# pjmikkol/bwtc

Hardware: NVIDIA B200
Metric: forward BWT MB/s (SA+BWT, 32 MiB blocks) (higher is better)
Workload: dtype u8 text / u32 ranks / u64 sort keys (integer)

## Files before the change

bwtc_b200/csrc/bwt_engine.cu:

```cuda
#include "../../include/bwtc_cuda.h"
#include "bwt_kernels.cuh"
#include "ibwt_kernels.cuh"

#include <algorithm>
#include <atomic>
#include <chrono>
#include <cmath>
#include <condition_variable>
#include <cstdarg>
#include <cstdio>
#include <cstdlib>
#include <cstring>
#include <deque>
#include <memory>
#include <mutex>
#include <thread>
#include <unordered_map>
#include <vector>

using namespace bwtc_b200;

namespace {

constexpr int RS_BLOCK = BWTC_RS_BLOCK;
// ... 46 lines not shown
  bool ring_busy[RING_SLOTS] = {false, false, false, false};
  int poll_spin_us = 150, poll_sleep_us = 40;
  int wait_mode = 0;
  uint32_t cap = 0;
  size_t max_rs_tiles = 0, max_aux_tiles = 0;
  uint8_t* d_in = nullptr;
  uint8_t* d_text = nullptr;
  uint8_t* d_out = nullptr;
  uint32_t* d_rank = nullptr;
  void* d_keys[2] = {nullptr, nullptr};
  uint32_t* d_idx[2] = {nullptr, nullptr};
  uint8_t* d_aux[2] = {nullptr, nullptr};
  uint32_t* d_scat = nullptr;
  uint32_t* d_zero = nullptr;
  uint32_t* d_status = nullptr;
  uint32_t* d_tilecnt = nullptr;
  uint32_t* d_LF = nullptr;
  uint32_t* d_livebits = nullptr;
  uint32_t* d_ktab = nullptr;
  LookupParams* d_lookup = nullptr;
  LookupParams* h_lookup = nullptr;
  LadderState* d_state = nullptr;
  LadderState* h_state = nullptr;
  unsigned long long* d_wtab = nullptr;
  uint32_t* d_bhist = nullptr;
  const uint8_t** d_bptr = nullptr;
  int32_t* d_sa = nullptr;
  uint32_t* h_small = nullptr;
  uint8_t* h_batch = nullptr;
  cudaEvent_t ev_begin = nullptr, ev_end = nullptr;
  std::vector<cudaEvent_t> ev_pool;
  int timing_detail = 0;
  int static_tiles = 1;
  int lb_watchdog = 0;
  int debug_fake_watchdog = 0;
  int debug_reverse_tiles = 0;
  int verify = 0;
  int debug_corrupt_out = 0;
  uint32_t debug_corrupt_lf = 0;
  int64_t debug_corrupt_sa = -1;
  int d2h_kernel = 0;
  int d2h_ctas = 16;
  int debug_skip_copies = 0;
  int ladder_first = 2, ladder_more = 4;
  int use_radix9 = 0;
  uint32_t status_row_words = 256;
  int use_partial = 1;
  int use_gram = 1;
  int twopass = 0;
  int hybrid2 = 0;
  uint32_t rerank_pf_tiles = 0;
  int use_lazy = 1;
  uint32_t lazy_min_suffixes = 4u << 20;
  double lazy_max_live = 0.065;
  int use_seg = 1;
  int use_batch = 1;
  int use_pack_pred = 1;
  uint32_t aux_min_suffixes = 96u << 20;
  int bucket_min_windows = 3;
  uint64_t rerank_window_bytes = 72ull << 20;
  uint32_t force_chars = 0, force_keybytes = 0;
  uint32_t debug_max_rounds = 0;
  int last_cur = 0;
  RerankParams rr0;
  bwtc_cuda_stats stats;
  char err[512];
  uint32_t* d_ctrl() const { return d_zero; }
  uint32_t* d_hist() const { return d_zero + CTR_WORDS; }
  unsigned long long* d_tstate() const { return reinterpret_cast<unsigned long long*>(d_zero + CTR_WORDS + HIST_WORDS); }
  uint32_t* h_ctrl() const { return h_small; }
  uint32_t* h_hist() const { return h_small + CTR_WORDS; }
  uint32_t* h_LF() const { return h_small + CTR_WORDS + HIST_WORDS; }
};

#define CK(ctx, call)                                                                              \
  do {                                                                                             \
    cudaError_t e_ = (call);                                                                       \
    if (e_ != cudaSuccess) {                                                                       \
      set_err((ctx)->err, "CUDA error %s at %s:%d: %s", cudaGetErrorName(e_), __FILE__, __LINE__,  \
              cudaGetErrorString(e_));                                                             \
      return BWTC_CUDA_ECUDA;                                                                      \
    }                                                                                              \
  } while (0)

namespace {

template <typename KeyT, int IPT, bool IOTA, bool AUX, int RB = 8>
int set_pass_attr(bwtc_cuda_ctx* ctx) {
  CK(ctx, cudaFuncSetAttribute(k_radix_pass<KeyT, RS_BLOCK, IPT, IOTA, AUX, RB>, cudaFuncAttributeMaxDynamicSharedMemorySize,
                               (int)RadixPassSmem<KeyT, RS_BLOCK, IPT, AUX, RB>::bytes));
  return 0;
}

void ctx_free(bwtc_cuda_ctx* c) {
  if (!c) return;
  cudaSetDevice(c->device);
  if (c->stream) cudaStreamSynchronize(c->stream);
  cudaFree(c->d_in); cudaFree(c->d_text); cudaFree(c->d_out); cudaFree(c->d_rank);
  cudaFree(c->d_keys[0]); cudaFree(c->d_keys[1]); cudaFree(c->d_idx[0]); cudaFree(c->d_idx[1]);
  cudaFree(c->d_zero); cudaFree(c->d_status); cudaFree(c->d_LF); cudaFree(c->d_wtab); cudaFree(c->d_tilecnt); cudaFree(c->d_scat);
  cudaFree(c->d_bhist); cudaFree(c->d_bptr); cudaFree(c->d_aux[0]); cudaFree(c->d_aux[1]);
  cudaFree(c->d_state); cudaFree(c->d_livebits); cudaFree(c->d_ktab); cudaFree(c->d_lookup); cudaFree(c->d_sa);
  if (c->h_lookup) cudaFreeHost(c->h_lookup);
  if (c->h_batch) cudaFreeHost(c->h_batch);
  if (c->h_small) cudaFreeHost(c->h_small);
  if (c->h_state) cudaFreeHost(c->h_state);
  if (c->h_ring) cudaFreeHost(c->h_ring);
  if (c->ev_begin) cudaEventDestroy(c->ev_begin);
  if (c->ev_end) cudaEventDestroy(c->ev_end);
  if (c->ev_sync) cudaEventDestroy(c->ev_sync);
  if (c->ev_in) cudaEventDestroy(c->ev_in);
  if (c->ev_comp) cudaEventDestroy(c->ev_comp);
  for (cudaEvent_t e : c->ev_ring) if (e) cudaEventDestroy(e);
  for (cudaEvent_t e : c->ev_pool) cudaEventDestroy(e);
  if (c->s_in) cudaStreamDestroy(c->s_in);
  if (c->s_out) cudaStreamDestroy(c->s_out);
  if (c->stream) cudaStreamDestroy(c->stream);
  delete c;
}

struct Round0Plan {
  uint32_t sigma, bits, chars, keybytes, npass;
  uint32_t rb;
  uint32_t rbits;
  PackParams pp;
  bool has_memory;
  double live_pred;
};

void plan_round0(const bwtc_cuda_ctx* ctx, const uint64_t* count, const bool* present, uint32_t N,
                 const double* pair_stats, Round0Plan* pl, uint32_t blk_bits = 0) {
  uint32_t sigma = blk_bits ? 1u : 0u;
  double total = 0, H0 = 0;
  for (int c = 0; c < 256; ++c) {
    pl->pp.lut[c] = 0;
    if (present[c]) { pl->pp.lut[c] = (uint8_t)sigma; ++sigma; total += (double)count[c]; }
  }
  if (sigma > 256) sigma = 256;
  for (int c = 0; c < 256; ++c)
    if (present[c] && count[c]) { double p = (double)count[c] / total; H0 -= p * std::log2(p); }
  const uint32_t b = sigma <= 2 ? 1 : ceil_log2_u64(sigma);
  const uint32_t cmax64 = (64 - blk_bits) / b, cmax32 = blk_bits >= 32 - b ? 0u : (32 - blk_bits) / b;
  uint32_t chars, keybytes;
  if (ctx->force_chars || ctx->force_keybytes) {
    keybytes = (ctx->force_keybytes == 4 && cmax32 >= 1) ? 4 : 8;
    const uint32_t cmax = keybytes == 4 ? cmax32 : cmax64;
    chars = ctx->force_chars ? ctx->force_chars : cmax;
    if (chars > cmax) chars = cmax;
    if (chars < 1) chars = 1;
  } else {
    double q2 = 0.0;
    for (int c = 0; c < 256; ++c)
      if (present[c] && count[c]) { const double q = (double)count[c] / total; q2 += q * q; }
    const double samples = pair_stats[1];
    const double all_pairs = samples * (samples - 1.0) * 0.5;
    const double expected = all_pairs * std::pow(q2, 8.0);
    const bool has_memory = (H0 < 1e-3) || samples < 64.0 || (pair_stats[0] > 8.0 * expected + 16.0);
    if (has_memory) {
      keybytes = 8;
      chars = cmax64;
    } else {
      const double npd = std::ceil((2.0 * std::log2((double)N + 2.0)) / 8.0);
      double best = 1e300;
      chars = cmax64;
      for (uint32_t c = 1; c <= cmax64; ++c) {
        const double p0 = std::ceil(((double)c * b + blk_bits) / 8.0) * ((uint64_t)c * b + blk_bits > 32 ? 1.1 : 1.0);
        const double L = 1.0 - std::exp(-(double)N * std::exp2(-H0 * (double)c));
        const double cost = p0 + L * (npd + 2.0);
        if (cost < best - 1e-9) { best = cost; chars = c; }
      }
      const uint32_t np = div_up((uint64_t)chars * b + blk_bits, 8);
      const uint32_t cfull = (8 * np - blk_bits) / b;
      const uint32_t cap = ((uint64_t)chars * b + blk_bits <= 32) ? cmax32 : cmax64;
      chars = cfull < cap ? cfull : cap;
      keybytes = ((uint64_t)chars * b + blk_bits <= 32) ? 4 : 8;
    }
  }
  pl->has_memory = true;
  pl->live_pred = 1.0;
  if (!(ctx->force_chars || ctx->force_keybytes)) {
    double q2 = 0.0;
    for (int c = 0; c < 256; ++c)
      if (present[c] && count[c]) { const double q = (double)count[c] / total; q2 += q * q; }
    const double samples = pair_stats[1];
    const double expected = samples * (samples - 1.0) * 0.5 * std::pow(q2, 8.0);
    pl->has_memory = (H0 < 1e-3) || samples < 64.0 || (pair_stats[0] > 8.0 * expected + 16.0);
    if (!pl->has_memory) pl->live_pred = 1.0 - std::exp(-(double)N * std::exp2(-H0 * (double)chars));
  }
  pl->sigma = sigma;
  pl->bits = b;
  pl->chars = chars;
  pl->keybytes = keybytes;
  pl->npass = div_up((uint64_t)chars * b + blk_bits, 8);
  pl->rb = 8;
  if (ctx->use_radix9 && keybytes == 8 && div_up((uint64_t)chars * b + blk_bits, 9) < pl->npass) {
    pl->rb = 9;
    pl->npass = div_up((uint64_t)chars * b + blk_bits, 9);
  }
  {
    const uint32_t covered = std::min<uint32_t>(pl->rb * pl->npass, keybytes * 8u);
    const uint32_t used = chars * b + blk_bits;
    uint32_t r = (ctx->use_partial && blk_bits == 0 && covered > used) ? covered - used : 0u;
    if (r >= b) r = b - 1u;
    if (chars >= 64u) r = 0;
    pl->rbits = r;
  }
  pl->pp.rbits = pl->rbits;
  pl->pp.bits = b;
  pl->pp.chars = chars;
  pl->pp.nblocks = 1;
  pl->pp.stride = 0;
}

uint32_t rerank_windows(const bwtc_cuda_ctx* ctx, uint32_t N, uint32_t m) {
  if ((uint64_t)m * 4 < (uint64_t)N) return 1;
  uint64_t w = ((uint64_t)N * 4 + ctx->rerank_window_bytes - 1) / ctx->rerank_window_bytes;
  if (w < 1) w = 1;
  if (!ctx->bucket_min_windows && w > 8) w = 8;
  if (w > MAX_RERANK_WINDOWS) w = MAX_RERANK_WINDOWS;
  return (uint32_t)w;
}

uint32_t rerank_launches(const bwtc_cuda_ctx* ctx, uint32_t N, uint32_t m) {
  const uint32_t w = rerank_windows(ctx, N, m);
  return (ctx->bucket_min_windows && w >= (uint32_t)ctx->bucket_min_windows) ? 1u : w;
}

inline bool dbg_any(const bwtc_cuda_ctx* ctx) { return ctx->debug_max_rounds != 0; }

inline uint32_t tile_slot(const bwtc_cuda_ctx* ctx, uint32_t ticket_word) {
  if (!ctx->static_tiles) return ticket_word;
  return ctx->debug_reverse_tiles ? CTR_STATIC_REV : CTR_STATIC;
}

inline uint32_t* status_rows(const bwtc_cuda_ctx* ctx, int p) {
  return ctx->d_status + ((size_t)p * (ctx->max_rs_tiles + LB_PAD_ROWS) + LB_PAD_ROWS) * ctx->status_row_words;
}

struct PassTimer {
  bwtc_cuda_ctx* ctx;
// ... 517 lines not shown
        }
        if (sft >= 32u) use_gram = false;
        gp.u[p] = (uint8_t)u;
        gp.s[p] = (uint8_t)sft;
      }
      gp.npass = pl.npass;
    }
    uint32_t* gram = use_gram ? ctx->d_hist() + GRAM_OFF : nullptr;
    if (use_gram) { hist_mask = 0; dp.count = 0; }
    if (pl.keybytes == 4) {
      k_pack_round0<uint32_t><<<grid, 256, 0, st>>>(d_text, N, static_cast<uint32_t*>(ctx->d_keys[0]), pl.pp,
                                                     ctx->d_hist(), hist_mask, ptiles, pl.rb, gram);
      if (dp.count) k_hist_derive<uint32_t><<<dp.count, 256, 0, st>>>(d_text, N, pl.pp, dp, ctx->d_hist(), pl.rb);
      if (use_gram) k_hist_from_gram<uint32_t><<<gp.npass, 256, 0, st>>>(d_text, N, pl.pp, gp, gram, ctx->d_hist(), pl.rb);
    } else {
      k_pack_round0<unsigned long long><<<grid, 256, 0, st>>>(d_text, N, static_cast<unsigned long long*>(ctx->d_keys[0]),
                                                               pl.pp, ctx->d_hist(), hist_mask, ptiles, pl.rb, gram);
      if (dp.count) k_hist_derive<unsigned long long><<<dp.count, 256, 0, st>>>(d_text, N, pl.pp, dp, ctx->d_hist(), pl.rb);
      if (use_gram)
        k_hist_from_gram<unsigned long long><<<gp.npass, 256, 0, st>>>(d_text, N, pl.pp, gp, gram, ctx->d_hist(), pl.rb);
    }
    if (dp.count || use_gram) S.kernel_launches++;
    CK(ctx, cudaGetLastError());
    S.kernel_launches++;
    S.algorithmic_bytes += (uint64_t)N + (uint64_t)N * pl.keybytes;
  }
  const uint32_t mask0 = all0;
  int cur = 0;
  uint32_t pdone = 0;
  int rc;
  uint32_t id_bits = (uint32_t)ceil_log2_u64((uint64_t)N);
  if (id_bits < 1) id_bits = 1;
  const bool pack_pred = ctx->use_pack_pred && (id_bits + pl.bits <= 32) && (mask0 & 1u);
  const uint32_t topshift = (pl.chars - 1) * pl.bits + pl.rbits;
  const uint32_t pred_mask = (1u << pl.bits) - 1u;
  const bool aux_pred = !pack_pred && ctx->aux_min_suffixes && N >= ctx->aux_min_suffixes && (mask0 & 1u) && !bs;
  if (pl.keybytes == 4)
    rc = run_sort<uint32_t, RS_IPT32>(ctx, N, mask0, true, N - 1, &cur, &pt, &pdone, pack_pred ? id_bits : 0u, topshift,
                                      pred_mask, aux_pred);
  else
    rc = run_sort<unsigned long long, RS_IPT64>(ctx, N, mask0, true, N - 1, &cur, &pt, &pdone, pack_pred ? id_bits : 0u,
                                                topshift, pred_mask, aux_pred, pl.rb);
  if (rc) return rc;
  const size_t round0_events = pt.used;
  S.sort0_launches = S.sort_launches;
  S.sort0_bytes = S.sort_bytes;
  S.live[0] = N;
  S.passes[0] = pdone;
  S.prefix_len[0] = 0;
  S.rounds = 1;
  bool lazy = false;
  const uint32_t keybits0 = pl.chars * pl.bits + pl.rbits;
  if (ctx->use_lazy && !bs && !dbg_any(ctx) && N >= 64 && keybits0 >= 1) {
    lazy = ctx->use_lazy >= 2 || (!pl.has_memory && pl.live_pred <= ctx->lazy_max_live && N >= ctx->lazy_min_suffixes);
  }
  const uint32_t tbits = std::min<uint32_t>(KTAB_BITS, keybits0);
  const uint32_t lazy_cap = N / 6;
  {
    RerankParams rp;
    rp.m = N;
    {
      const uint32_t text_end = J.sentinel_outside_alphabet ? N - 1 : N;
      const uint32_t wchars = pl.chars + (pl.rbits ? 1u : 0u);
      rp.short_thresh = wchars > text_end ? 0u : text_end - wchars + 1u;
    }
    rp.lo_bits = 0;
    rp.lazy = lazy ? 1u : 0u;
    rp.livebits = ctx->d_livebits;
    rp.ktab = ctx->d_ktab;
    rp.tshift = keybits0 - tbits;
    if (lazy) {
      CK(ctx, cudaMemsetAsync(ctx->d_livebits, 0, ((size_t)N / 32 + 4) * 4, st));
      CK(ctx, cudaMemsetAsync(ctx->d_ktab, 0xFF, ((size_t)(1u << tbits) + 2) * 4, st));
      LookupParams& L = *ctx->h_lookup;
      L.enabled = 1;
      L.keybytes = pl.keybytes;
      L.sorted_keys = ctx->d_keys[cur];
      L.ktab = ctx->d_ktab;
      L.livebits = ctx->d_livebits;
      L.text = d_text;
      L.N = N;
      L.bits = pl.bits;
      L.chars = pl.chars;
      L.rbits = pl.rbits;
      L.tshift = keybits0 - tbits;
      memcpy(L.lut, pl.pp.lut, 256);
      CK(ctx, cudaMemcpyAsync(ctx->d_lookup, ctx->h_lookup, sizeof(LookupParams), cudaMemcpyHostToDevice, st));
    }
    S.flags = (ctx->static_tiles ? 0u : 1u) | (bs ? 2u : 0u) | (pack_pred ? 4u : 0u) | (aux_pred ? 8u : 0u) | (lazy ? 16u : 0u) |
              (J.sa ? 256u : 0u);
    rp.packed = pack_pred ? 1u : (aux_pred ? 2u : 0u);
    rp.pred_aux = ctx->d_aux[cur];
    rp.id_bits = pack_pred ? id_bits : 31u;
    rp.id_mask = pack_pred ? (uint32_t)((1ull << id_bits) - 1ull) : 0xFFFFFFFFu;
    memset(rp.decode, 0, sizeof(rp.decode));
    for (int c = 0; c < 256; ++c)
      if (J.present[c]) rp.decode[pl.pp.lut[c]] = (uint8_t)c;
    uint32_t* snr = reinterpret_cast<uint32_t*>(ctx->d_keys[cur ^ 1]);
    if (pl.keybytes == 4) rc = launch_rerank<uint32_t, true>(ctx, cur, N, N, rp, ep, snr, snr + N, lazy);
    else rc = launch_rerank<unsigned long long, true>(ctx, cur, N, N, rp, ep, snr, snr + N, lazy);
    if (rc) return rc;
    S.algorithmic_bytes += (uint64_t)N * (pl.keybytes + 4) + (lazy ? 0ull : (uint64_t)N * 4);
    if (lazy) {
      const uint32_t entries = 1u << tbits, nchunks = div_up(entries, KTAB_CHUNK);
      uint32_t* cmin = ctx->d_bhist;
      k_ktab_chunkmin<<<nchunks, 256, 0, st>>>(ctx->d_ktab, entries, cmin);
      k_ktab_fill<<<nchunks, 256, 0, st>>>(ctx->d_ktab, entries, N, cmin, nchunks);
// ... 818 lines not shown
    set_err(g_err, "cudaGetDeviceCount: %s", cudaGetErrorString(e));
    return BWTC_CUDA_ECUDA;
  }
  return n;
}

#define BWTC_STR2(x) #x
#define BWTC_STR(x) BWTC_STR2(x)
const char* bwtc_cuda_version(void) {
  return "bwtc_b200 0.1 sm_100a radix-pass BLOCK=" BWTC_STR(BWTC_RS_BLOCK) " IPT64=" BWTC_STR(BWTC_RS_IPT64)
         " IPT32=" BWTC_STR(BWTC_RS_IPT32);
}

const char* bwtc_cuda_global_error(void) { return g_err; }

uint32_t bwtc_cuda_stats_sizeof(void) { return (uint32_t)sizeof(bwtc_cuda_stats); }

int bwtc_cuda_ctx_create(bwtc_cuda_ctx** out, int device, uint32_t max_block_bytes) {
  if (!out || max_block_bytes == 0) { set_err(g_err, "bad arguments"); return BWTC_CUDA_EARG; }
  if (max_block_bytes > BWTC_CUDA_MAX_BLOCK) { set_err(g_err, "max_block_bytes above engine limit"); return BWTC_CUDA_ETOOBIG; }
  *out = nullptr;
  cudaError_t e = cudaSetDevice(device);
  if (e != cudaSuccess) { set_err(g_err, "cudaSetDevice(%d): %s", device, cudaGetErrorString(e)); return BWTC_CUDA_ECUDA; }
  bwtc_cuda_ctx* c = new (std::nothrow) bwtc_cuda_ctx();
  if (!c) { set_err(g_err, "out of host memory"); return BWTC_CUDA_EALLOC; }
  c->device = device;
  c->cap = max_block_bytes;
  if (const char* e = getenv("BWTC_STATIC_TILES")) c->static_tiles = atoi(e);
  if (const char* e = getenv("BWTC_DEBUG_FAKE_WATCHDOG")) c->debug_fake_watchdog = atoi(e);
  if (const char* e = getenv("BWTC_DEBUG_REVERSE_TILES")) c->debug_reverse_tiles = atoi(e);
  if (const char* e = getenv("BWTC_VERIFY")) c->verify = atoi(e) ? 1 : 0;
  if (const char* e = getenv("BWTC_DEBUG_CORRUPT_OUT")) c->debug_corrupt_out = atoi(e);
  if (const char* e = getenv("BWTC_DEBUG_CORRUPT_LF")) c->debug_corrupt_lf = (uint32_t)std::max(0, atoi(e));
  if (const char* e = getenv("BWTC_DEBUG_CORRUPT_SA")) c->debug_corrupt_sa = std::max(-1L, atol(e));
  if (const char* e = getenv("BWTC_DEBUG_SKIP_COPIES")) c->debug_skip_copies = atoi(e);
  if (const char* e = getenv("BWTC_D2H_KERNEL")) c->d2h_kernel = atoi(e);
  if (const char* e = getenv("BWTC_D2H_CTAS")) c->d2h_ctas = std::max(1, atoi(e));
  if (const char* e = getenv("BWTC_SPIN_WAIT")) c->wait_mode = atoi(e) ? 1 : 0;
  if (const char* e = getenv("BWTC_WAIT_MODE")) c->wait_mode = atoi(e);
  if (const char* e = getenv("BWTC_POLL_SPIN_US")) c->poll_spin_us = std::max(0, atoi(e));
  if (const char* e = getenv("BWTC_POLL_SLEEP_US")) c->poll_sleep_us = std::max(1, atoi(e));
  if (const char* e = getenv("BWTC_LADDER_FIRST")) c->ladder_first = std::max(0, atoi(e));
  if (const char* e = getenv("BWTC_LADDER_MORE")) c->ladder_more = std::max(1, atoi(e));
  if (const char* e = getenv("BWTC_LAZY")) c->use_lazy = atoi(e);
  if (const char* e = getenv("BWTC_HYBRID2")) c->hybrid2 = atoi(e);
  if (const char* e = getenv("BWTC_TWOPASS")) c->twopass = atoi(e);
  if (const char* e = getenv("BWTC_GRAM")) c->use_gram = atoi(e);
  if (const char* e = getenv("BWTC_PARTIAL")) c->use_partial = atoi(e);
  if (const char* e = getenv("BWTC_RERANK_PF")) c->rerank_pf_tiles = (uint32_t)std::max(0, atoi(e));
  c->use_radix9 = env_radix9();
  c->status_row_words = status_row_words_for(c->use_radix9);
  if (const char* e = getenv("BWTC_LAZY_MIN_MIB")) c->lazy_min_suffixes = (uint32_t)std::max(0L, atol(e)) << 20;
  if (const char* e = getenv("BWTC_LAZY_MAX_LIVE")) c->lazy_max_live = atof(e);
  if (const char* e = getenv("BWTC_SEG")) c->use_seg = atoi(e);
  if (const char* e = getenv("BWTC_BATCH")) c->use_batch = atoi(e);
  if (const char* e = getenv("BWTC_PACK_PRED")) c->use_pack_pred = atoi(e);
  if (const char* e = getenv("BWTC_AUX_MIN_MIB")) { const long v = atol(e); c->aux_min_suffixes = v > 0 ? (uint32_t)v << 20 : (v == 0 ? 1u : 0u); }
  if (const char* e = getenv("BWTC_BUCKET_MIN_WINDOWS")) c->bucket_min_windows = atoi(e);
  if (const char* e = getenv("BWTC_RERANK_WINDOW_MB")) { long v = atol(e); if (v > 0) c->rerank_window_bytes = (uint64_t)v << 20; }
  c->err[0] = 0;
  memset(&c->stats, 0, sizeof(c->stats));
  const size_t N = (size_t)max_block_bytes + 1;
  const uint32_t min_tile = RS_TILE64 < RS_TILE32 ? RS_TILE64 : RS_TILE32;
  c->max_rs_tiles = div_up(N, min_tile);
  c->max_aux_tiles = div_up(N, AUX_TILE);
  int rc = 0;
#define ALLOC(ptr, bytes)                                                                       \
  do {                                                                                          \
    if (!rc) {                                                                                  \
      e = cudaMalloc((void**)&(ptr), (bytes));                                                  \
      if (e != cudaSuccess) {                                                                   \
        set_err(g_err, "cudaMalloc(%zu bytes) for " #ptr ": %s", (size_t)(bytes), cudaGetErrorString(e)); \
        rc = BWTC_CUDA_EALLOC;                                                                  \
      }                                                                                         \
    }                                                                                           \
  } while (0)
  int sm = 0;
  if (cudaDeviceGetAttribute(&sm, cudaDevAttrMultiProcessorCount, device) == cudaSuccess && sm > 0) c->sm_count = sm;
  {
    size_t free_b = 0, total_b = 0;
    const uint64_t need = bwtc_cuda_scratch_bytes(max_block_bytes);
    if (cudaMemGetInfo(&free_b, &total_b) == cudaSuccess && need > (uint64_t)free_b) {
      set_err(g_err, "a context for %u-byte blocks needs %llu bytes of device memory, %llu are free", max_block_bytes,
              (unsigned long long)need, (unsigned long long)free_b);
      delete c;
      return BWTC_CUDA_EALLOC;
    }
  }
  e = cudaStreamCreateWithFlags(&c->stream, cudaStreamNonBlocking);
  if (e != cudaSuccess) { set_err(g_err, "cudaStreamCreate: %s", cudaGetErrorString(e)); rc = BWTC_CUDA_ECUDA; }
  const size_t padded = ((N + TEXT_PAD + 15) / 16) * 16 + 16;
  ALLOC(c->d_in, padded);
  ALLOC(c->d_text, padded);
  ALLOC(c->d_out, padded);
  ALLOC(c->d_rank, (N + 64) * 4);
  ALLOC(c->d_keys[0], N * 8 + 64);
  ALLOC(c->d_keys[1], N * 8 + 64);
  ALLOC(c->d_idx[0], N * 4);
  ALLOC(c->d_idx[1], N * 4);
  ALLOC(c->d_zero, (size_t)(CTR_WORDS + HIST_WORDS) * 4 + (size_t)MAX_RERANK_WINDOWS * c->max_aux_tiles * 8 + 64);
  ALLOC(c->d_status, (size_t)MAX_PASSES * (c->max_rs_tiles + LB_PAD_ROWS) * c->status_row_words * 4u);
  ALLOC(c->d_LF, (size_t)LF_WORDS * 4);
  ALLOC(c->d_state, sizeof(LadderState));
  ALLOC(c->d_livebits, (N / 32 + 4) * 4);
  ALLOC(c->d_ktab, ((size_t)(1u << KTAB_BITS) + 2) * 4);
  ALLOC(c->d_lookup, sizeof(LookupParams));
// ... 629 lines not shown
```

bwtc_b200/csrc/bwt_kernels.cuh:

```cuda
#pragma once
#include <cuda_runtime.h>
#include <stdint.h>

namespace bwtc_b200 {

constexpr uint32_t RANK_DONE = 0x80000000u;
constexpr uint32_t RANK_MASK = 0x7FFFFFFFu;

constexpr int CTR_ERR = 0;
constexpr int CTR_STICKY = 8;
constexpr int CTR_PASS0 = 8;
constexpr uint32_t CTR_STATIC = 0xFFFFFFFFu;
constexpr uint32_t CTR_STATIC_REV = 0xFFFFFFFEu;
constexpr int CTR_CURSOR = 24;
constexpr int CTR_LIVE = 25;
constexpr int CTR_MAXGROUP = 26;
constexpr int CTR_UPD = 27;
constexpr int CTR_RERANK = 32;
constexpr int MAX_RERANK_WINDOWS = 16;
constexpr int CTR_WORDS = 64;

constexpr uint32_t LB_PREFIX = 0x80000000u, LB_VALUE = 0x7FFFFFFFu;
constexpr uint32_t LB_PAD_WORD = LB_PREFIX | 1u;
__constant__ uint32_t g_lb_spin_limit = 1u << 24;
// ... 928 lines not shown
  uint32_t* ktab;
  uint32_t tshift;
};

struct LookupParams {
  uint32_t enabled;
  uint32_t keybytes;
  const void* sorted_keys;
  const uint32_t* ktab;
  const uint32_t* livebits;
  const uint8_t* text;
  uint32_t N, bits, chars, tshift;
  uint32_t rbits;
  uint8_t lut[256];
};

template <typename KeyT>
__device__ __forceinline__ uint32_t sector_lower_bound(const KeyT* __restrict__ sk, KeyT key, uint32_t lo, uint32_t hi,
                                                       uint32_t frac16) {
  constexpr uint32_t KPS = 32 / sizeof(KeyT);
  uint32_t g = lo + (uint32_t)(((unsigned long long)(hi - lo) * frac16) >> 16);
  for (int it = 0; lo < hi; ++it) {
    if (g >= hi) g = hi - 1u;
    if (g < lo) g = lo;
    const uint32_t s = g & ~(KPS - 1u);
    KeyT v[KPS];
    if constexpr (sizeof(KeyT) == 8) {
      const ulonglong2 x = *reinterpret_cast<const ulonglong2*>(sk + s);
      const ulonglong2 y = *reinterpret_cast<const ulonglong2*>(sk + s + 2);
      v[0] = (KeyT)x.x; v[1] = (KeyT)x.y; v[2] = (KeyT)y.x; v[3] = (KeyT)y.y;
    } else {
      const uint4 x = *reinterpret_cast<const uint4*>(sk + s);
      const uint4 y = *reinterpret_cast<const uint4*>(sk + s + 4);
      v[0] = (KeyT)x.x; v[1] = (KeyT)x.y; v[2] = (KeyT)x.z; v[3] = (KeyT)x.w;
      v[4] = (KeyT)y.x; v[5] = (KeyT)y.y; v[6] = (KeyT)y.z; v[7] = (KeyT)y.w;
    }
    const uint32_t a = s > lo ? s : lo, b = (s + KPS < hi) ? s + KPS : hi;
    uint32_t c = 0;
#pragma unroll
    for (uint32_t q = 0; q < KPS; ++q) c += (s + q >= a && s + q < b && v[q] < key) ? 1u : 0u;
    if (c == 0u) {
      hi = a;
      g = (it < 2) ? (a ? a - 1u : 0u) : lo + ((hi - lo) >> 1);
    } else if (c == b - a) {
      lo = b;
      g = (it < 2) ? b : lo + ((hi - lo) >> 1);
    } else {
      return a + c;
    }
  }
  return lo;
}

__device__ __forceinline__ uint32_t rank_lookup(const LookupParams& lk, const uint32_t* __restrict__ rank, uint32_t j) {
  if (!lk.enabled || ((lk.livebits[j >> 5] >> (j & 31u)) & 1u)) return rank[j] & RANK_MASK;
  unsigned long long key = 0;
  for (uint32_t c = 0; c < lk.chars; ++c) {
    const uint32_t g = j + c;
    key = (key << lk.bits) | (unsigned long long)((g < lk.N) ? lk.lut[lk.text[g]] : 0u);
  }
  if (lk.rbits) {
    const uint32_t g = j + lk.chars;
    key = (key << lk.rbits) | (unsigned long long)(((g < lk.N) ? (uint32_t)lk.lut[lk.text[g]] : 0u) >> (lk.bits - lk.rbits));
  }
  const uint32_t p = (uint32_t)(key >> lk.tshift);
  uint32_t lo = lk.ktab[p], hi = lk.ktab[p + 1u];
#ifndef BWTC_LAZY_BINSEARCH
  const uint32_t frac16 = lk.tshift >= 16u ? (uint32_t)(key >> (lk.tshift - 16u)) & 0xFFFFu
                                           : ((uint32_t)key << (16u - lk.tshift)) & 0xFFFFu;
  if (lk.keybytes == 8u)
    return sector_lower_bound<unsigned long long>(static_cast<const unsigned long long*>(lk.sorted_keys), key, lo, hi, frac16);
  return sector_lower_bound<uint32_t>(static_cast<const uint32_t*>(lk.sorted_keys), (uint32_t)key, lo, hi, frac16);
#else
  if (lk.keybytes == 8u) {
    const unsigned long long* sk = static_cast<const unsigned long long*>(lk.sorted_keys);
    while (lo < hi) {
      const uint32_t mid = lo + ((hi - lo) >> 1);
      if (sk[mid] < key) lo = mid + 1u; else hi = mid;
    }
  } else {
    const uint32_t* sk = static_cast<const uint32_t*>(lk.sorted_keys);
    const uint32_t k32 = (uint32_t)key;
    while (lo < hi) {
      const uint32_t mid = lo + ((hi - lo) >> 1);
      if (sk[mid] < k32) lo = mid + 1u; else hi = mid;
    }
  }
  return lo;
#endif
}

constexpr uint32_t KTAB_CHUNK = 4096;

__global__ void __launch_bounds__(256) k_ktab_chunkmin(const uint32_t* __restrict__ ktab, uint32_t entries, uint32_t* __restrict__ cmin) {
  __shared__ uint32_t s_w[8];
  const uint32_t base = blockIdx.x * KTAB_CHUNK + threadIdx.x * 16u;
  uint32_t mn = 0xFFFFFFFFu;
#pragma unroll
  for (int k = 0; k < 16; ++k)
    if (base + k < entries) mn = min(mn, ktab[base + k]);
#pragma unroll
  for (int o = 16; o > 0; o >>= 1) mn = min(mn, __shfl_xor_sync(0xFFFFFFFFu, mn, o));
  if ((threadIdx.x & 31) == 0) s_w[threadIdx.x >> 5] = mn;
  __syncthreads();
  if (threadIdx.x == 0) {
    uint32_t t = 0xFFFFFFFFu;
    for (int w = 0; w < 8; ++w) t = min(t, s_w[w]);
    cmin[blockIdx.x] = t;
  }
}

__global__ void __launch_bounds__(256) k_ktab_fill(uint32_t* __restrict__ ktab, uint32_t entries, uint32_t N,
                                                   const uint32_t* __restrict__ cmin, uint32_t nchunks) {
  __shared__ uint32_t s_w[8];
  __shared__ uint32_t s_carry;
  const int tid = threadIdx.x, lane = tid & 31, warp = tid >> 5;
  uint32_t c = N;
  for (uint32_t q = blockIdx.x + 1u + tid; q < nchunks; q += 256) c = min(c, cmin[q]);
#pragma unroll
  for (int o = 16; o > 0; o >>= 1) c = min(c, __shfl_xor_sync(0xFFFFFFFFu, c, o));
  if (lane == 0) s_w[warp] = c;
  __syncthreads();
  if (tid == 0) {
    uint32_t t = N;
    for (int w = 0; w < 8; ++w) t = min(t, s_w[w]);
    s_carry = t;
    if (blockIdx.x == nchunks - 1u) ktab[entries] = N;
  }
  __syncthreads();
  const uint32_t carry = s_carry;
  const uint32_t base = blockIdx.x * KTAB_CHUNK + (uint32_t)tid * 16u;
  uint32_t v[16];
  uint32_t mn = 0xFFFFFFFFu;
#pragma unroll
  for (int k = 0; k < 16; ++k) {
    v[k] = (base + k < entries) ? ktab[base + k] : 0xFFFFFFFFu;
    mn = min(mn, v[k]);
  }
  uint32_t inc = mn;
#pragma unroll
  for (int o = 1; o < 32; o <<= 1) {
    const uint32_t t = __shfl_down_sync(0xFFFFFFFFu, inc, o);
// ... 639 lines not shown
  const uint32_t wanted = st ? st->lists : 1u, err = ctrl[CTR_ERR];
  const uint32_t c = cnt[tile], dst = excl[tile];
  if (!wanted || err) return;
  const size_t src = (size_t)tile * tile_records;
  for (uint32_t t = threadIdx.x; t < c; t += blockDim.x) {
    out_nr[dst + t] = stage_nr[src + t];
    out_id[dst + t] = stage_id[src + t];
  }
}

__global__ void __launch_bounds__(256) k_build_from_list(const uint32_t* __restrict__ list, uint32_t m,
                                                         const uint32_t* __restrict__ rank, uint32_t N, uint32_t h,
                                                         int lo_bits, unsigned long long* __restrict__ keys,
                                                         uint32_t* __restrict__ idx, uint32_t* __restrict__ hist,
                                                         int npass, const uint32_t* __restrict__ ctrl, uint32_t rb) {
  __shared__ uint32_t s_hist[8 * 512];
  const int tid = threadIdx.x;
  const uint32_t dmask = (1u << rb) - 1u;
  if (ctrl[CTR_ERR]) return;
#pragma unroll
  for (int p = 0; p < 16; ++p) s_hist[p * 256 + tid] = 0;
  __syncthreads();
  for (uint32_t j = blockIdx.x * blockDim.x + tid; j < m; j += gridDim.x * blockDim.x) {
    const uint32_t i = list[j];
    const uint32_t r = rank[i] & RANK_MASK;
    const uint32_t r2 = (h < N - i) ? ((rank[i + h] & RANK_MASK) + 1u) : 0u;
    const unsigned long long key = ((unsigned long long)(r >> 1) << lo_bits) | (unsigned long long)r2;
    keys[j] = key;
    idx[j] = i | ((r & 1u) << 31);
    for (int p = 0; p < npass; ++p) atomicAdd(&s_hist[(p << rb) + ((uint32_t)(key >> (rb * p)) & dmask)], 1u);
  }
  __syncthreads();
  for (int p = 0; p < npass; ++p)
    for (uint32_t e = tid; e <= dmask; e += 256) {
      const uint32_t v = s_hist[(p << rb) + e];
      if (v) atomicAdd(&hist[(p << rb) + e], v);
    }
}

#ifndef BWTC_SEG_MINB
#define BWTC_SEG_MINB 4
#endif

#ifndef BWTC_SEG_MINB_LAZY
#define BWTC_SEG_MINB_LAZY 4
#endif
template <bool LAZY, bool SA = false>
__global__ void __launch_bounds__(256, LAZY ? BWTC_SEG_MINB_LAZY : BWTC_SEG_MINB) k_seg_round(const LadderState* __restrict__ st, PoolPtrs pool,
                                                   const uint32_t* __restrict__ rank, uint32_t N, EmitParams ep,
                                                   uint32_t* __restrict__ ctrl, const LookupParams* __restrict__ lkp) {
  constexpr int IPT = SEG_CAP / 256;
  __shared__ unsigned long long s_key[SEG_CAP];
  __shared__ uint32_t s_id[SEG_CAP];
  __shared__ uint32_t s_wa[8], s_wb[8];
  __shared__ uint32_t s_start, s_end, s_base;
  const int tid = threadIdx.x, lane = tid & 31, warp = tid >> 5;
  const uint32_t m_in = st->m, h = st->h, st_maxgroup = st->maxgroup, st_lists = st->lists, err = ctrl[CTR_ERR];
  if (!(st_lists && m_in > (uint32_t)SMALL_MAX && st_maxgroup <= (uint32_t)SEG_MAXGROUP) || err) return;
  __shared__ uint32_t* s_ptr[6];
  if (tid == 0) {
    int fslot[4];
    ladder_free_slots(st->sel, fslot);
    s_ptr[0] = pool.p[st->sel & 15u];
    s_ptr[1] = pool.p[st->sel >> 4];
    for (int q = 0; q < 4; ++q) s_ptr[2 + q] = pool.p[fslot[q]];
  }
#define nr_in (static_cast<const uint32_t*>(s_ptr[0]))
#define id_in (static_cast<const uint32_t*>(s_ptr[1]))
#define nr_out (s_ptr[2])
#define id_out (s_ptr[3])
#define upd_id (s_ptr[4])
#define upd_nr (s_ptr[5])
  for (uint32_t a = blockIdx.x * (uint32_t)SEG_T; a < m_in; a += gridDim.x * (uint32_t)SEG_T) {
  __syncthreads();
  const uint32_t b = (m_in - a > (uint32_t)SEG_T) ? a + SEG_T : m_in;
  if (tid == 0) { s_start = 0xFFFFFFFFu; s_end = (b >= m_in) ? m_in : 0xFFFFFFFFu; }
  __syncthreads();
  for (uint32_t t = tid; t <= (uint32_t)SEG_MAXGROUP; t += 256) {
    const uint32_t ja = a + t;
    if (ja < m_in) {
      if (ja == 0 || nr_in[ja] != nr_in[ja - 1]) atomicMin(&s_start, ja);
    } else if (ja == m_in) {
      atomicMin(&s_start, m_in);
    }
    const uint32_t jb = b + t;
    if (b < m_in) {
      if (jb < m_in) {
        if (nr_in[jb] != nr_in[jb - 1]) atomicMin(&s_end, jb);
      } else if (jb == m_in) {
        atomicMin(&s_end, m_in);
      }
    }
  }
  __syncthreads();
  const uint32_t start = s_start, end = s_end;
  if (start == 0xFFFFFFFFu || end == 0xFFFFFFFFu || (start < end && end - start > (uint32_t)SEG_CAP)) {
    if (tid == 0) atomicExch(&ctrl[CTR_ERR], 4u);
    continue;
  }
  if (start >= end) continue;
  uint32_t myid[IPT], mynr[IPT];
  uint32_t livemask = 0;
#pragma unroll
  for (int k = 0; k < IPT; ++k) {
    const uint32_t j = start + tid * IPT + k;
    mynr[k] = RANK_DONE;
    myid[k] = 0;
    if (j < end) { mynr[k] = nr_in[j]; myid[k] = id_in[j]; }
    if (!(mynr[k] & RANK_DONE)) livemask |= 1u << k;
  }
  uint32_t cnt = __popc(livemask), inc = cnt;
#pragma unroll
  for (int o = 1; o < 32; o <<= 1) {
    const uint32_t t = __shfl_up_sync(0xFFFFFFFFu, inc, o);
    if (lane >= o) inc += t;
  }
  if (lane == 31) s_wa[warp] = inc;
  __syncthreads();
  uint32_t woff = 0, L = 0;
#pragma unroll
  for (int w = 0; w < 8; ++w) { const uint32_t t = s_wa[w]; if (w < warp) woff += t; L += t; }
  {
    uint32_t lo[IPT];
    if (!LAZY) {
#pragma unroll
      for (int k = 0; k < IPT; ++k) {
        lo[k] = 0;
        if (((livemask >> k) & 1u) && h < N - myid[k]) lo[k] = (rank[myid[k] + h] & RANK_MASK) + 1u;
      }
    } else {
#pragma unroll
      for (int k = 0; k < IPT; ++k) {
        lo[k] = 0;
        if (((livemask >> k) & 1u) && h < N - myid[k]) lo[k] = rank_lookup(*lkp, rank, myid[k] + h) + 1u;
      }
    }
    uint32_t pos = woff + inc - cnt;
#pragma unroll
    for (int k = 0; k < IPT; ++k) {
      if ((livemask >> k) & 1u) {
        s_key[pos] = ((unsigned long long)mynr[k] << 32) | lo[k];
        s_id[pos] = myid[k];
        ++pos;
      }
    }
  }
  __syncthreads();
  if (L == 0) continue;
  const uint32_t P = L;
  {
    unsigned long long kreg[IPT];
    uint32_t ireg[IPT], npos[IPT];
#pragma unroll
    for (int k = 0; k < IPT; ++k) {
      const uint32_t j = (uint32_t)tid + 256u * k;
      npos[k] = 0xFFFFFFFFu;
      if (j < L) {
        kreg[k] = s_key[j];
        ireg[k] = s_id[j];
        const uint32_t g = (uint32_t)(kreg[k] >> 32);
        uint32_t cntb = 0, gs = j;
        for (uint32_t q = j; q-- > 0;) {
          const unsigned long long kq = s_key[q];
          if ((uint32_t)(kq >> 32) != g) break;
          cntb += (kq <= kreg[k]) ? 1u : 0u;
          gs = q;
        }
        for (uint32_t q = j + 1; q < L; ++q) {
          const unsigned long long kq = s_key[q];
          if ((uint32_t)(kq >> 32) != g) break;
          cntb += (kq < kreg[k]) ? 1u : 0u;
        }
        npos[k] = gs + cntb;
      }
    }
    __syncthreads();
#pragma unroll
    for (int k = 0; k < IPT; ++k) {
      if (npos[k] != 0xFFFFFFFFu) {
        s_key[npos[k]] = kreg[k];
        s_id[npos[k]] = ireg[k];
      }
    }
    __syncthreads();
  }
  unsigned long long key[IPT];
  uint32_t runf = 0, runh = 0, lf[IPT], lh[IPT], hfmask = 0;
  const uint32_t j0 = tid * IPT;
#pragma unroll
  for (int k = 0; k < IPT; ++k) {
    const uint32_t j = j0 + k;
    key[k] = (j < P) ? s_key[j] : ~0ull;
    myid[k] = (j < P) ? s_id[j] : 0u;
    const unsigned long long pk = (j > 0 && j <= P) ? s_key[j - 1] : 0ull;
    const bool hf = (j == 0) || (j >= L) || (key[k] != pk);
    const bool hh = (j == 0) || (j >= L) || ((key[k] >> 32) != (pk >> 32));
    if (hf) { hfmask |= 1u << k; runf = j + 1; }
    if (hh) runh = j + 1;
    lf[k] = runf;
    lh[k] = runh;
  }
  const unsigned long long nextkey = (j0 + IPT < P) ? s_key[j0 + IPT] : ~0ull;
  uint32_t incf = runf, inch = runh;
#pragma unroll
  for (int o = 1; o < 32; o <<= 1) {
    const uint32_t tf = __shfl_up_sync(0xFFFFFFFFu, incf, o), th = __shfl_up_sync(0xFFFFFFFFu, inch, o);
    if (lane >= o) { incf = max(incf, tf); inch = max(inch, th); }
  }
  uint32_t exf = __shfl_up_sync(0xFFFFFFFFu, incf, 1), exh = __shfl_up_sync(0xFFFFFFFFu, inch, 1);
  if (lane == 0) { exf = 0; exh = 0; }
  __syncthreads();
  if (lane == 31) { s_wa[warp] = incf; s_wb[warp] = inch; }
  __syncthreads();
  for (int w = 0; w < warp; ++w) { exf = max(exf, s_wa[w]); exh = max(exh, s_wb[w]); }
  uint32_t keep = 0, updm = 0, newnr[IPT], gmax = 0;
#pragma unroll
  for (int k = 0; k < IPT; ++k) {
    const uint32_t j = j0 + k;
    newnr[k] = 0;
    if (j < L) {
      const uint32_t HF = max(lf[k], exf) - 1u, HH = max(lh[k], exh) - 1u;
      const unsigned long long nk = (k == IPT - 1) ? nextkey : key[k + 1];
      const bool single = ((hfmask >> k) & 1u) && (j + 1 >= L || nk != key[k]);
      uint32_t nr = (uint32_t)(key[k] >> 32) + (HF - HH);
// ... 344 lines not shown
```

Baseline: 13590.

## Compare lazy rerank keys by round-0 prefix in segment sort, widen lazy gating

In the lazy segment-sort kernel, each suffix's rank lookup is replaced by its round-0 key plus the rank only when the suffix is live. Keys are compared as (round0 key, rank) pairs, and the in-group count of smaller entries becomes the new key. This removes the binary search into the sorted key table on every lazy lookup, at the cost of extra shared memory for the round-0 keys and heavier comparisons. Lazy mode is also enabled for texts with memory when the estimated repeats and the character count allow it, and the live threshold is raised, so more inputs take the lazy path.

```diff
diff --git a/bwtc_b200/csrc/bwt_engine.cu b/bwtc_b200/csrc/bwt_engine.cu
--- a/bwtc_b200/csrc/bwt_engine.cu
+++ b/bwtc_b200/csrc/bwt_engine.cu
@@ -122,7 +122,8 @@
   uint32_t rerank_pf_tiles = 0;
   int use_lazy = 1;
   uint32_t lazy_min_suffixes = 4u << 20;
-  double lazy_max_live = 0.065;
+  double lazy_max_live = 0.09;
+  double lazy_max_repeats = 32.0;
   int use_seg = 1;
   int use_batch = 1;
   int use_pack_pred = 1;
@@ -196,6 +197,7 @@
   PackParams pp;
   bool has_memory;
   double live_pred;
+  double repeats;
 };
 
 void plan_round0(const bwtc_cuda_ctx* ctx, const uint64_t* count, const bool* present, uint32_t N,
@@ -248,14 +250,17 @@
   }
   pl->has_memory = true;
   pl->live_pred = 1.0;
+  pl->repeats = HUGE_VAL;
   if (!(ctx->force_chars || ctx->force_keybytes)) {
     double q2 = 0.0;
     for (int c = 0; c < 256; ++c)
       if (present[c] && count[c]) { const double q = (double)count[c] / total; q2 += q * q; }
     const double samples = pair_stats[1];
-    const double expected = samples * (samples - 1.0) * 0.5 * std::pow(q2, 8.0);
+    const double all_pairs = samples * (samples - 1.0) * 0.5;
+    const double expected = all_pairs * std::pow(q2, 8.0);
     pl->has_memory = (H0 < 1e-3) || samples < 64.0 || (pair_stats[0] > 8.0 * expected + 16.0);
     if (!pl->has_memory) pl->live_pred = 1.0 - std::exp(-(double)N * std::exp2(-H0 * (double)chars));
+    if (samples >= 64.0) pl->repeats = pair_stats[0] / all_pairs * (double)N;
   }
   pl->sigma = sigma;
   pl->bits = b;
@@ -879,7 +884,10 @@
   bool lazy = false;
   const uint32_t keybits0 = pl.chars * pl.bits + pl.rbits;
   if (ctx->use_lazy && !bs && !dbg_any(ctx) && N >= 64 && keybits0 >= 1) {
-    lazy = ctx->use_lazy >= 2 || (!pl.has_memory && pl.live_pred <= ctx->lazy_max_live && N >= ctx->lazy_min_suffixes);
+    constexpr uint32_t LAZY_MIN_CHARS = 10;
+    const bool memory_ok = ctx->use_seg && pl.chars >= LAZY_MIN_CHARS && pl.repeats <= ctx->lazy_max_repeats;
+    lazy = ctx->use_lazy >= 2 ||
+           (N >= ctx->lazy_min_suffixes && (pl.has_memory ? memory_ok : pl.live_pred <= ctx->lazy_max_live));
   }
   const uint32_t tbits = std::min<uint32_t>(KTAB_BITS, keybits0);
   const uint32_t lazy_cap = N / 6;
@@ -1804,6 +1812,7 @@
   c->status_row_words = status_row_words_for(c->use_radix9);
   if (const char* e = getenv("BWTC_LAZY_MIN_MIB")) c->lazy_min_suffixes = (uint32_t)std::max(0L, atol(e)) << 20;
   if (const char* e = getenv("BWTC_LAZY_MAX_LIVE")) c->lazy_max_live = atof(e);
+  if (const char* e = getenv("BWTC_LAZY_MAX_REPEATS")) c->lazy_max_repeats = atof(e);
   if (const char* e = getenv("BWTC_SEG")) c->use_seg = atoi(e);
   if (const char* e = getenv("BWTC_BATCH")) c->use_batch = atoi(e);
   if (const char* e = getenv("BWTC_PACK_PRED")) c->use_pack_pred = atoi(e);
diff --git a/bwtc_b200/csrc/bwt_kernels.cuh b/bwtc_b200/csrc/bwt_kernels.cuh
--- a/bwtc_b200/csrc/bwt_kernels.cuh
+++ b/bwtc_b200/csrc/bwt_kernels.cuh
@@ -1004,8 +1004,7 @@
   return lo;
 }
 
-__device__ __forceinline__ uint32_t rank_lookup(const LookupParams& lk, const uint32_t* __restrict__ rank, uint32_t j) {
-  if (!lk.enabled || ((lk.livebits[j >> 5] >> (j & 31u)) & 1u)) return rank[j] & RANK_MASK;
+__device__ __forceinline__ unsigned long long round0_key(const LookupParams& lk, uint32_t j) {
   unsigned long long key = 0;
   for (uint32_t c = 0; c < lk.chars; ++c) {
     const uint32_t g = j + c;
@@ -1015,31 +1014,19 @@
     const uint32_t g = j + lk.chars;
     key = (key << lk.rbits) | (unsigned long long)(((g < lk.N) ? (uint32_t)lk.lut[lk.text[g]] : 0u) >> (lk.bits - lk.rbits));
   }
+  return key;
+}
+
+__device__ __forceinline__ uint32_t rank_lookup(const LookupParams& lk, const uint32_t* __restrict__ rank, uint32_t j) {
+  if (!lk.enabled || ((lk.livebits[j >> 5] >> (j & 31u)) & 1u)) return rank[j] & RANK_MASK;
+  const unsigned long long key = round0_key(lk, j);
   const uint32_t p = (uint32_t)(key >> lk.tshift);
   uint32_t lo = lk.ktab[p], hi = lk.ktab[p + 1u];
-#ifndef BWTC_LAZY_BINSEARCH
   const uint32_t frac16 = lk.tshift >= 16u ? (uint32_t)(key >> (lk.tshift - 16u)) & 0xFFFFu
                                            : ((uint32_t)key << (16u - lk.tshift)) & 0xFFFFu;
   if (lk.keybytes == 8u)
     return sector_lower_bound<unsigned long long>(static_cast<const unsigned long long*>(lk.sorted_keys), key, lo, hi, frac16);
   return sector_lower_bound<uint32_t>(static_cast<const uint32_t*>(lk.sorted_keys), (uint32_t)key, lo, hi, frac16);
-#else
-  if (lk.keybytes == 8u) {
-    const unsigned long long* sk = static_cast<const unsigned long long*>(lk.sorted_keys);
-    while (lo < hi) {
-      const uint32_t mid = lo + ((hi - lo) >> 1);
-      if (sk[mid] < key) lo = mid + 1u; else hi = mid;
-    }
-  } else {
-    const uint32_t* sk = static_cast<const uint32_t*>(lk.sorted_keys);
-    const uint32_t k32 = (uint32_t)key;
-    while (lo < hi) {
-      const uint32_t mid = lo + ((hi - lo) >> 1);
-      if (sk[mid] < k32) lo = mid + 1u; else hi = mid;
-    }
-  }
-  return lo;
-#endif
 }
 
 constexpr uint32_t KTAB_CHUNK = 4096;
@@ -1785,6 +1772,7 @@
   constexpr int IPT = SEG_CAP / 256;
   __shared__ unsigned long long s_key[SEG_CAP];
   __shared__ uint32_t s_id[SEG_CAP];
+  __shared__ unsigned long long s_k0[LAZY ? SEG_CAP : 1];
   __shared__ uint32_t s_wa[8], s_wb[8];
   __shared__ uint32_t s_start, s_end, s_base;
   const int tid = threadIdx.x, lane = tid & 31, warp = tid >> 5;
@@ -1853,26 +1841,37 @@
   uint32_t woff = 0, L = 0;
 #pragma unroll
   for (int w = 0; w < 8; ++w) { const uint32_t t = s_wa[w]; if (w < warp) woff += t; L += t; }
-  {
+  if constexpr (!LAZY) {
     uint32_t lo[IPT];
-    if (!LAZY) {
-#pragma unroll
-      for (int k = 0; k < IPT; ++k) {
-        lo[k] = 0;
-        if (((livemask >> k) & 1u) && h < N - myid[k]) lo[k] = (rank[myid[k] + h] & RANK_MASK) + 1u;
-      }
-    } else {
-#pragma unroll
-      for (int k = 0; k < IPT; ++k) {
-        lo[k] = 0;
-        if (((livemask >> k) & 1u) && h < N - myid[k]) lo[k] = rank_lookup(*lkp, rank, myid[k] + h) + 1u;
-      }
+#pragma unroll
+    for (int k = 0; k < IPT; ++k) {
+      lo[k] = 0;
+      if (((livemask >> k) & 1u) && h < N - myid[k]) lo[k] = (rank[myid[k] + h] & RANK_MASK) + 1u;
     }
     uint32_t pos = woff + inc - cnt;
 #pragma unroll
     for (int k = 0; k < IPT; ++k) {
       if ((livemask >> k) & 1u) {
         s_key[pos] = ((unsigned long long)mynr[k] << 32) | lo[k];
+        s_id[pos] = myid[k];
+        ++pos;
+      }
+    }
+  } else {
+    uint32_t pos = woff + inc - cnt;
+#pragma unroll
+    for (int k = 0; k < IPT; ++k) {
+      if ((livemask >> k) & 1u) {
+        unsigned long long k0 = 0;
+        uint32_t lo = 0;
+        if (h < N - myid[k]) {
+          const uint32_t j = myid[k] + h;
+          const uint32_t lw = lkp->livebits[j >> 5];
+          k0 = round0_key(*lkp, j);
+          lo = ((lw >> (j & 31u)) & 1u) ? (rank[j] & RANK_MASK) + 1u : 0xFFFFFFFFu;
+        }
+        s_key[pos] = ((unsigned long long)mynr[k] << 32) | lo;
+        s_k0[pos] = k0;
         s_id[pos] = myid[k];
         ++pos;
       }
@@ -1893,16 +1892,40 @@
         ireg[k] = s_id[j];
         const uint32_t g = (uint32_t)(kreg[k] >> 32);
         uint32_t cntb = 0, gs = j;
-        for (uint32_t q = j; q-- > 0;) {
-          const unsigned long long kq = s_key[q];
-          if ((uint32_t)(kq >> 32) != g) break;
-          cntb += (kq <= kreg[k]) ? 1u : 0u;
-          gs = q;
-        }
-        for (uint32_t q = j + 1; q < L; ++q) {
-          const unsigned long long kq = s_key[q];
-          if ((uint32_t)(kq >> 32) != g) break;
-          cntb += (kq < kreg[k]) ? 1u : 0u;
+        if constexpr (!LAZY) {
+          for (uint32_t q = j; q-- > 0;) {
+            const unsigned long long kq = s_key[q];
+            if ((uint32_t)(kq >> 32) != g) break;
+            cntb += (kq <= kreg[k]) ? 1u : 0u;
+            gs = q;
+          }
+          for (uint32_t q = j + 1; q < L; ++q) {
+            const unsigned long long kq = s_key[q];
+            if ((uint32_t)(kq >> 32) != g) break;
+            cntb += (kq < kreg[k]) ? 1u : 0u;
+          }
+        } else {
+          const unsigned long long k0 = s_k0[j];
+          const uint32_t lo = (uint32_t)kreg[k];
+          uint32_t nlt = 0;
+          for (uint32_t q = j; q-- > 0;) {
+            const unsigned long long kq = s_key[q];
+            if ((uint32_t)(kq >> 32) != g) break;
+            const unsigned long long k0q = s_k0[q];
+            const bool lt = k0q < k0 || (k0q == k0 && (uint32_t)kq < lo);
+            nlt += lt ? 1u : 0u;
+            cntb += (lt || (k0q == k0 && (uint32_t)kq == lo)) ? 1u : 0u;
+            gs = q;
+          }
+          for (uint32_t q = j + 1; q < L; ++q) {
+            const unsigned long long kq = s_key[q];
+            if ((uint32_t)(kq >> 32) != g) break;
+            const unsigned long long k0q = s_k0[q];
+            const bool lt = k0q < k0 || (k0q == k0 && (uint32_t)kq < lo);
+            nlt += lt ? 1u : 0u;
+            cntb += lt ? 1u : 0u;
+          }
+          kreg[k] = ((unsigned long long)g << 32) | nlt;
         }
         npos[k] = gs + cntb;
       }
```

After: 14790 (median of 6 runs). +8.8%, better.
